# TGoldC/Motion-Planning-for-Autonomous-Driving-with-MPC

Measured on AMD Instinct MI355X. Metric: MPC steps/sec (N=30, nx=6 nu=2) at batch=4096, higher is better.
Workload: dtype f64; 1 GPU; N=30 nx=6 nu=2 bicycle lane-following, batch=4096/GPU, tol 1e-8; mode=converged, gpu=AMD Radeon Graphics

## Files before the change

motion-planning-for-autonomous-driving-with-mpc_amd/csrc/mpc_host_common.h:

```cpp
#pragma once
#include <cmath>
#include <cstddef>
#include <cstdint>
#include <cstdio>
#include <string>
#include <utility>
#include <vector>

#include "../../include/mpcgpu.h"
#include "mpc_stage_math.h"

namespace mpc {

constexpr double BOUND_RELAX = 1e-8;
constexpr int SENS_NWT = 7, SENS_NWQ = 5;
constexpr int LOOP_NS = 5, LOOP_NPOSE = 3;

struct HostProblem {
    mpc_problem_desc desc{};
    std::vector<double> LB, UB;
    int has_fl = 0, has_fu = 0, has_ol = 0, has_ou = 0;
    double fl = 0, fu = 0, ol = 0, ou = 0;
    double ol_raw = 0;
    double fl_raw = 0;
// ... 146 lines not shown
    w.MZU = w.total; w.total += mb * NZ;
    w.MSO = w.total; w.total += mb * 4;
    w.MNUO = w.total; w.total += mb * 4;
    w.MZLO = w.total; w.total += mb * 4;
    w.MZUO = w.total; w.total += mb * 4;
    w.MLAM = w.total; w.total += mb * XS;
    w.MREF = w.total; w.total += mb * XS;
    w.itotal = w.ntiles * w.itile_elems;
    return w;
}

inline int pick_bx(int N, int max_threads) {
    int bx = 64;
    while (bx > 4 && bx * (N + 1) > max_threads) bx >>= 1;
    return bx;
}

inline int dec_s_of(const HostProblem& hp) {
    return (hp.desc.nx == 6 && hp.desc.Q[5] == 0.0 && !((hp.lo_mask | hp.hi_mask) & (1u << 7))) ? 1 : 0;
}

inline void fill_params(Params& P, const HostProblem& hp, int B, size_t Bp, int bx, double* base, int32_t* ibase,
                        const double* dLB, const double* dUB, bool mailbox = true, int obst_stages = 0) {
    const mpc_problem_desc& d = hp.desc;
    const WsLayout w = ws_layout(d.N, d.nx, Bp, mailbox, obst_stages);
    P.B = B; P.Bp = (int32_t)Bp; P.N = d.N; P.nx = d.nx; P.bx = bx;
    P.obst_mult = d.obst_mult; P.max_iter = d.max_iter; P.fixed_iters = d.fixed_iters;
    P.has_fl = hp.has_fl; P.has_fu = hp.has_fu; P.has_ol = hp.has_ol; P.has_ou = hp.has_ou; P.per_inst_obst = OBST_SHARED;
    P.dt = d.dt; P.wheelbase = d.wheelbase; P.friction_div = d.friction_div; P.ego_offset = d.ego_offset; P.tol = d.tol;
    for (int i = 0; i < 6; ++i) P.Q[i] = (i < d.nx) ? d.Q[i] : 0.0;
    P.R[0] = d.R[0]; P.R[1] = d.R[1];
    for (int i = 0; i < 6; ++i) P.obst[i] = d.obstacle[i];
    P.fl = hp.fl; P.fu = hp.fu; P.ol = hp.ol; P.ou = hp.ou;
    P.inv_S = (uint32_t)((0x100000000ull + (uint64_t)d.N) / (uint64_t)(d.N + 1));
    P.run_counter = nullptr;
    P.dec_s = 0;
    P.tile_mask = nullptr;
    P.lo_mask = hp.lo_mask; P.hi_mask = hp.hi_mask; P.dense_mask = hp.dense_mask;
    P.dec_s = dec_s_of(hp);
    P.x0 = nullptr; P.p = nullptr; P.LB = dLB; P.UB = dUB;
    P.Z = base + w.Z * 64; P.ZL = base + w.ZL * 64; P.ZU = base + w.ZU * 64;
    P.SO = base + w.SO * 64; P.NUO = base + w.NUO * 64; P.ZLO = base + w.ZLO * 64; P.ZUO = base + w.ZUO * 64;
    P.LAM = base + w.LAM * 64; P.REF = base + w.REF * 64; P.DZ = base + w.DZ * 64; P.PK = base + w.PK * 64; P.KK = base + w.KK * 64;
    P.BLK = base + w.BLK * 64; P.ROLL = base + w.ROLL * 64; P.SC = base + w.SC * 64;
    P.FILT = base + w.FILT * 64; P.OBST = base + w.OBST * 64;
    P.MBLK = base + w.MBLK; P.MPK = base + w.MPK; P.MDZ = base + w.MDZ;
    P.MZ = base + w.MZ; P.MZL = base + w.MZL; P.MZU = base + w.MZU; P.MSO = base + w.MSO; P.MNUO = base + w.MNUO; P.MZLO = base + w.MZLO;
    P.MZUO = base + w.MZUO; P.MLAM = base + w.MLAM; P.MREF = base + w.MREF;
    P.tile_elems = (uint32_t)w.tile_elems; P.itile_elems = (uint32_t)w.itile_elems;
    P.ISC = ibase;
    P.WS = base; P.IWS = ibase;
    P.ws_bytes = (uint32_t)(w.total * sizeof(double)); P.iws_bytes = (uint32_t)(w.itotal * sizeof(int32_t));
    P.x_out = nullptr; P.status_out = nullptr; P.iters_out = nullptr; P.kkt_out = nullptr;
    P.emit = 0; P.fail_count = nullptr; P.fin_ctl = nullptr; P.fin_host = nullptr;
    P.DBG = nullptr;
    P.tile0 = 0;
}

inline void default_desc(mpc_problem_desc* d, int32_t N, int32_t nx) {
    *d = mpc_problem_desc{};
    d->N = N; d->nx = nx; d->nu = 2; d->formulation = MPC_FORM_CASADI_EULER;
    d->max_iter = 100; d->fixed_iters = 0; d->obst_mult = 3; d->device = 0;
    d->dt = 0.1; d->wheelbase = 2.5789128; d->friction_div = 2.578; d->ego_offset = 0.75; d->tol = 1e-8;
    const double Q[5] = {2.3, 2.3, 500.0, 0.1, 10.0};
    for (int i = 0; i < 5; ++i) d->Q[i] = Q[i];
    d->R[0] = 2.0; d->R[1] = 0.2;
    const double Pt[5] = {80.0, 80.0, 100.0, 0.1, 100.0};
    for (int i = 0; i < 5; ++i) d->P[i] = Pt[i];
    for (int j = 0; j < 3; ++j) { d->obstacle[2 * j] = -100.0; d->obstacle[2 * j + 1] = 0.0; }
}

}
```

motion-planning-for-autonomous-driving-with-mpc_amd/csrc/mpc_solve_plan.h:

```cpp
#pragma once
#include <algorithm>
#include <cctype>
#include <cstdlib>
#include <cstring>
#include <string>

#include "mpc_host_common.h"

namespace mpc {

struct Knobs {
    int pipeline, hybrid, hybrid_bx, hybrid_live, pipe_help, pipe_test_abort, pipe_xcd_mask, pipe_early;
    int rescue, rescue_wg, rescue_alone, loop_async, sync_spin, max_batch, friction_lb, bound_mask, big_wg, groups, poison;
    int timing;
    Knobs();
};
enum class KnobParse {
    ON,
    INT,
    FLAG,
    MASK,
    FRIC,
};
struct KnobDef { const char* name; int Knobs::*field; int dflt; KnobParse parse; };
inline constexpr KnobDef KNOBS[] = {
    {"pipeline", &Knobs::pipeline, 1, KnobParse::ON},           {"hybrid", &Knobs::hybrid, 1, KnobParse::INT},
    {"hybrid_bx", &Knobs::hybrid_bx, 0, KnobParse::INT},        {"hybrid_live", &Knobs::hybrid_live, -1, KnobParse::INT},
    {"pipe_help", &Knobs::pipe_help, -1, KnobParse::INT},       {"pipe_test_abort", &Knobs::pipe_test_abort, 0, KnobParse::FLAG},
    {"pipe_xcd_mask", &Knobs::pipe_xcd_mask, 0, KnobParse::MASK}, {"rescue", &Knobs::rescue, 1, KnobParse::ON},
    {"rescue_wg", &Knobs::rescue_wg, 1, KnobParse::INT},        {"rescue_alone", &Knobs::rescue_alone, 0, KnobParse::FLAG},
    {"loop_async", &Knobs::loop_async, 1, KnobParse::ON},       {"sync_spin", &Knobs::sync_spin, 1, KnobParse::ON},
    {"max_batch", &Knobs::max_batch, 0, KnobParse::INT},        {"friction_lb", &Knobs::friction_lb, 0, KnobParse::FRIC},
    {"bound_mask", &Knobs::bound_mask, 1, KnobParse::INT},      {"big_wg", &Knobs::big_wg, 0, KnobParse::FLAG},
    {"groups", &Knobs::groups, 0, KnobParse::INT},              {"poison", &Knobs::poison, 0, KnobParse::FLAG},
    {"timing", &Knobs::timing, 0, KnobParse::INT},               {"pipe_early", &Knobs::pipe_early, -1, KnobParse::INT},
};
inline Knobs::Knobs() { for (const KnobDef& e : KNOBS) this->*e.field = e.dflt; }
inline const KnobDef* find_knob(const char* name) {
    for (const KnobDef& e : KNOBS) if (name && strcmp(name, e.name) == 0) return &e;
    return nullptr;
}
inline int set_knob(Knobs& k, const char* name, const char* value) {
    const KnobDef* e = find_knob(name);
    if (!e) return MPC_ERR_INVALID;
    int v = e->dflt;
    if (value) {
        const long iv = strtol(value, nullptr, 0);
        switch (e->parse) {
            case KnobParse::ON: v = value[0] != '0'; break;
            case KnobParse::INT: v = (int)iv; break;
            case KnobParse::FLAG: v = (value[0] == '\0' ? 1 : (int)iv) != 0; break;
            case KnobParse::MASK: v = (int)(uint32_t)strtoul(value, nullptr, 0); break;
            case KnobParse::FRIC: v = strcmp(value, "ipopt") == 0 ? 1 : strcmp(value, "nlp") == 0 ? 0 : (int)iv; break;
        }
    }
    k.*e->field = v;
    return MPC_OK;
}
inline int get_knob(const Knobs& k, const char* name, long* out) {
    const KnobDef* e = find_knob(name);
    if (!e) return MPC_ERR_INVALID;
    *out = e->parse == KnobParse::MASK ? (long)(uint32_t)(k.*e->field) : (long)(k.*e->field);
    return MPC_OK;
}
inline void knobs_from_env(Knobs& k) {
    for (const KnobDef& e : KNOBS) {
        std::string env = "MPCGPU_";
        for (const char* c = e.name; *c; ++c) env += (char)toupper(*c);
        const char* v = getenv(env.c_str());
        if (v) (void)set_knob(k, e.name, v);
    }
}

constexpr int TIMING_STAGE = 1,
              TIMING_PIPE = 2,
              TIMING_WG = 4,
              TIMING_START = 8,
              TIMING_WG_TRACE = 16;

constexpr int STAGE_MAX_THREADS = 512;
constexpr int MAX_GROUPS = 4;
constexpr int MAX_POLL_IT = 1024;
constexpr size_t LDS_MAX = 160 * 1024 - 1024;

#ifndef MPC_STAGE_STASH
#define MPC_STAGE_STASH 1
#endif
template <int NX> struct Stash {
// ... 297 lines not shown
```

motion-planning-for-autonomous-driving-with-mpc_amd/csrc/mpc_stage_math.h:

```cpp
#pragma once
#include <math.h>
#include <stdint.h>

#if defined(__HIPCC__)
#define MPC_HD __host__ __device__ __forceinline__
#else
#define MPC_HD inline
#endif

#if defined(__HIP_DEVICE_COMPILE__)
#define MPC_GLOBAL_AS __attribute__((address_space(1)))
#else
#define MPC_GLOBAL_AS
#endif
#define MPC_GP(ptr, idx) (((MPC_GLOBAL_AS __typeof__(*(ptr))*)(ptr))[(uint32_t)(idx)])

namespace mpc {

constexpr double MU_INIT = 0.1, KAPPA_EPS = 10.0, KAPPA_MU = 0.2, THETA_MU = 1.5, TAU_MIN = 0.99;
constexpr double KAPPA_1 = 1e-2, KAPPA_2 = 1e-2, S_MAX = 100.0, KAPPA_SIGMA = 1e10;
constexpr double GAMMA_THETA = 1e-5, GAMMA_PHI = 1e-8, LS_DELTA = 1.0, S_THETA = 1.1, S_PHI = 2.3;
constexpr double ETA_PHI = 1e-8, GAMMA_ALPHA = 0.05;
constexpr double DW_MIN = 1e-20, DW_0 = 1e-4, DW_MAX = 1e40, KW_MINUS = 1.0 / 3.0, KW_PLUS = 8.0, KW_PLUS_BAR = 100.0;
constexpr double SCALING_MAX_GRAD = 100.0;
// ... 25 lines not shown
    SC_COUNT
};
enum IsRow { IS_STATUS = 0, IS_ITERS, IS_NFILT, IS_HAVETH0, IS_CONV, IS_ROLL, IS_FROW,
             IS_ILL,
             IS_RLEV, IS_ITACC,
             IS_COUNT };
enum ObstMode : int32_t { OBST_SHARED = 0, OBST_PER_INSTANCE = 1, OBST_PER_STAGE = 2, OBST_PER_STAGE_SIZED = 3 };
MPC_HD constexpr bool obst_mode_staged(int32_t m) { return m == OBST_PER_STAGE || m == OBST_PER_STAGE_SIZED; }
struct Params {
    int32_t B, Bp, N, nx, bx;
    int32_t obst_mult, max_iter, fixed_iters;
    int32_t has_fl, has_fu, has_ol, has_ou;
    int32_t per_inst_obst;
    double dt, wheelbase, friction_div, ego_offset, tol;
    double Q[6], R[2], obst[6];
    double fl, fu, ol, ou;
    int32_t dec_s;
    unsigned long long* tile_mask;
    int32_t* run_counter;
    uint32_t inv_S;
    uint32_t dense_mask;
    uint32_t lo_mask, hi_mask;
    const double* x0;
    const double* p;
    const double* LB;
    const double* UB;
    double *Z, *ZL, *ZU;
    double *SO, *NUO, *ZLO, *ZUO;
    double *LAM;
    double *REF;
    double *DZ;
    double *PK;
    double *KK;
    double *BLK;
    double *ROLL;
    double *MBLK, *MPK, *MDZ;
    double *MZ, *MZL, *MZU, *MSO, *MNUO, *MZLO, *MZUO, *MLAM, *MREF;
    double *SC;
    double *FILT;
    const double* OBST;
    int32_t* ISC;
    double* WS;
    int32_t* IWS;
    uint32_t ws_bytes, iws_bytes;
    uint32_t tile_elems, itile_elems;
    int32_t tile0;
    int32_t mbw_live;
    unsigned long long* DBG;
    double* x_out;
    int32_t* status_out;
    int32_t* iters_out;
    double* kkt_out;
    int32_t emit;
    uint32_t* fail_count;
    uint32_t *fin_ctl, *fin_host;
};

#define MPC_EV(R) ((((uint32_t)(R)) + 1u) & ~1u)
MPC_HD constexpr uint32_t mpc_prow(uint32_t r) { return (r & ~1u) * 64u + (r & 1u); }
MPC_HD uint32_t ws_index(const Params& P, const double*, uint32_t row, uint32_t b) { return (b >> 6) * P.tile_elems + mpc_prow(row) + (b & 63u) * 2u; }
MPC_HD uint32_t ws_index(const Params& P, const int32_t*, uint32_t row, uint32_t b) { return (b >> 6) * P.itile_elems + mpc_prow(row) + (b & 63u) * 2u; }

#if defined(__HIP_DEVICE_COMPILE__)
typedef unsigned int mpc_v2u __attribute__((ext_vector_type(2)));
__host__ __device__ __forceinline__ __amdgpu_buffer_rsrc_t mpc_rsrc(const void* base, uint32_t bytes) {
    const uint64_t a = (uint64_t)(uintptr_t)base;
    uint32_t lo = (uint32_t)__builtin_amdgcn_readfirstlane((int)(uint32_t)a);
    uint32_t hi = (uint32_t)__builtin_amdgcn_readfirstlane((int)(uint32_t)(a >> 32));
    bytes = (uint32_t)__builtin_amdgcn_readfirstlane((int)bytes);
    asm("" : "+s"(lo), "+s"(hi), "+s"(bytes));
    return __builtin_amdgcn_make_buffer_rsrc((void*)(uintptr_t)(((uint64_t)hi << 32) | lo), 0, (int)bytes, 0x00020000);
}
__device__ __forceinline__ int mpc_uni(uint32_t v) { return __builtin_amdgcn_readfirstlane((int)v); }
constexpr int MPC_AUX_SC1 = 16;
struct DevParams : Params {
    __amdgpu_buffer_rsrc_t rws, riws;
    bool xcu;
    __host__ __device__ __forceinline__ explicit DevParams(const Params& q, const bool xcu_ = false)
        : Params(q), rws(mpc_rsrc(q.WS, q.ws_bytes)), riws(mpc_rsrc(q.IWS, q.iws_bytes)), xcu(xcu_) {}
};
typedef DevParams PRef;
__device__ __forceinline__ PRef mpc_pref(const Params& q, const bool xcu) { return DevParams(q, xcu); }
__device__ __forceinline__ mpc_v2u mpc_bload64(const DevParams& P, const __amdgpu_buffer_rsrc_t r, const int voff, const int soff) {
    return P.xcu ? __builtin_amdgcn_raw_buffer_load_b64(r, voff, soff, MPC_AUX_SC1) : __builtin_amdgcn_raw_buffer_load_b64(r, voff, soff, 0);
}
__device__ __forceinline__ unsigned mpc_bload32(const DevParams& P, const __amdgpu_buffer_rsrc_t r, const int voff, const int soff) {
    return P.xcu ? __builtin_amdgcn_raw_buffer_load_b32(r, voff, soff, MPC_AUX_SC1) : __builtin_amdgcn_raw_buffer_load_b32(r, voff, soff, 0);
}
struct WsRefD {
    const PRef& P;
    uint32_t aoff, uoff, voff;
    __device__ __forceinline__ operator double() const {
        const __amdgpu_buffer_rsrc_t r = P.rws;
        const mpc_v2u v = mpc_bload64(P, r, (int)voff, mpc_uni(aoff + uoff));
        return __builtin_bit_cast(double, v);
    }
    __device__ __forceinline__ double operator=(double x) const {
        __builtin_amdgcn_raw_buffer_store_b64(__builtin_bit_cast(mpc_v2u, x), P.rws, (int)voff, mpc_uni(aoff + uoff), 0);
        return x;
    }
    __device__ __forceinline__ double operator=(const WsRefD& o) const { return (*this = (double)o); }
};
struct WsRefI {
    const PRef& P;
    uint32_t soff, voff;
    __device__ __forceinline__ operator int32_t() const {
// ... 2079 lines not shown
```

motion-planning-for-autonomous-driving-with-mpc_amd/csrc/mpcgpu.hip:

```cpp
#include <hip/hip_runtime.h>
#include <type_traits>

#include <algorithm>
#include <cctype>
#include <cstdio>
#include <cstdlib>
#include <cstring>
#include <new>
#include <string>
#include <vector>

#include "mpc_host_common.h"
#include "mpc_solve_plan.h"
#include "mpc_stamps.h"
#include "mpc_closed_loop.h"
#include "mpc_forces_qp.h"
#include "mpc_riccati_mfma.h"
#include "mpc_sens.h"
#include "mpc_loop_lin.h"

using namespace mpc;

namespace {

__device__ __forceinline__ void lds_barrier() {
    asm volatile("s_waitcnt lgkmcnt(0)\n\ts_barrier" ::: "memory");
}
template <int MAXJ, class Load, class Store>
__device__ __forceinline__ void batched_fill(const int n, const int t, const int NT, Load ld, Store st) {
    for (int q0 = 0; q0 < n; q0 += MAXJ * NT) {
        double v[MAXJ];
#pragma unroll
        for (int j = 0; j < MAXJ; ++j) { const int q = q0 + j * NT + t; v[j] = (q < n) ? (double)ld(q) : 0.0; }
#pragma unroll
        for (int j = 0; j < MAXJ; ++j) { const int q = q0 + j * NT + t; if (q < n) st(q, v[j]); }
    }
}
template <int MAXJ>
__device__ __forceinline__ void fill_bounds(const PRef& P, double* tab, const int nb, const int t, const int NT) {
    batched_fill<2 * MAXJ>(2 * nb, t, NT, [&](int q) { return q < nb ? (double)MPC_GP(P.LB, q) : (double)MPC_GP(P.UB, q - nb); }, [&](int q, double v) { tab[q] = v; });
}

__device__ __forceinline__ uint32_t lds_uniform(const uint32_t v) { return (uint32_t)__builtin_amdgcn_readfirstlane((int)v); }
__device__ __forceinline__ int lds_uniform(const int v) { return __builtin_amdgcn_readfirstlane(v); }
__device__ __forceinline__ double lds_uniform(const double v) {
    const unsigned long long u = __builtin_bit_cast(unsigned long long, v);
    const unsigned long long r = ((unsigned long long)lds_uniform((uint32_t)(u >> 32)) << 32) | lds_uniform((uint32_t)u);
    return __builtin_bit_cast(double, r);
}

template <typename R>
__device__ __forceinline__ R shfl_xor_struct(const R& r, int mask) {
    constexpr int NQ = sizeof(R) / sizeof(double);
    R o;
    const double* s = reinterpret_cast<const double*>(&r);
    double* d = reinterpret_cast<double*>(&o);
#pragma unroll
    for (int i = 0; i < NQ; ++i) d[i] = __shfl_xor(s[i], mask, 64);
    return o;
}

template <typename R>
__device__ __forceinline__ void block_reduce(R& r, int bx, double* lds) {
    constexpr int NQ = sizeof(R) / sizeof(double);
    for (int m = bx; m < 64; m <<= 1) {
        const R o = shfl_xor_struct(r, m);
        red_combine(r, o);
    }
    const int nw = blockDim.x >> 6;
    if (nw > 1) {
        const int wave = threadIdx.x >> 6, lane = threadIdx.x & 63, bl = lane & (bx - 1);
        double* mine = reinterpret_cast<double*>(&r);
        if (lane < bx) {
#pragma unroll
            for (int q = 0; q < NQ; ++q) lds[(wave * NQ + q) * bx + lane] = mine[q];
        }
        lds_barrier();
        R acc;
        double* a = reinterpret_cast<double*>(&acc);
#pragma unroll
        for (int q = 0; q < NQ; ++q) a[q] = lds[q * bx + bl];
        for (int w = 1; w < nw; ++w) {
            R o;
            double* op = reinterpret_cast<double*>(&o);
#pragma unroll
            for (int q = 0; q < NQ; ++q) op[q] = lds[(w * NQ + q) * bx + bl];
            red_combine(acc, o);
        }
        r = acc;
        lds_barrier();
    }
}

typedef __attribute__((address_space(3))) void* lds_ptr_t;
template <int NX, bool OUT, uint32_t VM = 0xFFu>
__device__ __forceinline__ void stash_xfer(Ctx<NX>& c, double* st, int T, int t, bool has_ou) {
    int r = 0;
#define MPC_ST(v) do { if (OUT) st[r * T + t] = (v); else (v) = st[r * T + t]; ++r; } while (0)
#pragma unroll
    for (int i = 0; i < NX + 2; ++i) { if (!((VM >> i) & 1u)) continue; MPC_ST(c.zl[i]); MPC_ST(c.zu[i]); MPC_ST(c.igl[i]); MPC_ST(c.igu[i]); }
#pragma unroll
    for (int j = 0; j < 3; ++j) { MPC_ST(c.zlo[j]); MPC_ST(c.iglo[j]); }
    if (has_ou) {
#pragma unroll
        for (int j = 0; j < 3; ++j) { MPC_ST(c.zuo[j]); MPC_ST(c.iguo[j]); }
    }
#pragma unroll
    for (int j = 0; j < 3; ++j) MPC_ST(c.nuo[j]);
#pragma unroll
    for (int i = 0; i < NX; ++i) { MPC_ST(c.lam[i]); MPC_ST(c.dlam[i]); }
#undef MPC_ST
}

#ifndef MPC_REF_FLAGS
#define MPC_REF_FLAGS (VM_OSPEC | vm_dense(REF_DENSE_LO, REF_DENSE_HI))
#endif
constexpr uint32_t REF_VM = REF_BOUND_VM | MPC_REF_FLAGS;
constexpr uint32_t SIZED_VM = 0xFFu | VM_SIZED;
constexpr uint32_t var_vm(int var) { return var == 2 ? REF_VM : var == 4 ? SIZED_VM : 0xFFu; }
struct NoStepWait {
    __device__ __forceinline__ bool there() const { return true; }
    __device__ __forceinline__ bool operator()() const { return true; }
};
template <int NX, bool INIT, int MAXT, uint32_t VM = 0xFFu, class StepWait = NoStepWait, bool OSTG = true>
__device__ __forceinline__ void stage_block(const PRef& P, const int n_mult, const int n_z, const int stash_rows, const uint32_t b0,
                                            const unsigned long long tile_bits, double* lds, const bool stamp = true,
                                            uint32_t* live_out = nullptr, const bool bounds_in_lds = false, const StepWait& step_wait = StepWait()) {
    constexpr bool EARLY = !std::is_same<StepWait, NoStepWait>::value;
    static_assert(!(EARLY && INIT), "the start iterate reads no step");
    CtxOf<NX, VM> c;
    constexpr bool STASH = MAXT <= 256 && MPC_STAGE_STASH;
    const bool has_ou = (VM & VM_OSPEC) ? false : (P.has_ou != 0);
    const int bx = P.bx, t = threadIdx.x;
    c.k = t / bx;
    c.b = (int)b0 + (t & (bx - 1));
    c.valid = (c.k <= P.N) && (c.b < P.B);
    c.active = false;
    c.ill = false;
    c.status = 0;
    c.iters = 0;
    c.mbw = !INIT && P.mbw_live > 0 && __popcll(tile_bits) <= P.mbw_live;
    MPC_STAMP(P.DBG, blockIdx.x, SB_ENTER, t == 0 && stamp);
    if (!INIT) {
        const unsigned long long m = tile_bits >> (b0 & 63u);
        if ((m & ((bx >= 64) ? ~0ull : ((1ull << bx) - 1ull))) == 0ull) return;
    }
    double* lds_b = lds + (blockDim.x >> 6) * 10 * bx;
    const int nb = (P.N + 1) * (NX + 2);
    double* lds_x = lds_b + 2 * nb;
    if (!bounds_in_lds)
        fill_bounds<2>(P, lds_b, nb, t, (int)blockDim.x);
    c.bnd = (mpc_lds_cptr)(lds_ptr_t)lds_b;
    c.bnd_ub = nb;
    if (INIT) lds_barrier();
    if (INIT) {
        Red0 r0;
        phase_init_point<NX, OSTG, (VM & VM_SIZED) != 0u>(P, c, r0);
        block_reduce(r0, bx, lds);
        phase_init_scalars<NX>(P, c, r0);
    } else {
        phase_load_scalars<NX>(P, c);
        PreTmp<NX> tmp;
        if constexpr (EARLY) {
            phase_preload<NX, false, VM, true, false, false>(P, c, tmp);
            if (step_wait.there()) {
                phase_preload_step<NX>(P, c);
                MPC_STAMP(P.DBG, blockIdx.x, SB_ISSUED, t == 0 && stamp);
            } else {
                MPC_STAMP(P.DBG, blockIdx.x, SB_ISSUED, t == 0 && stamp);
                if (!step_wait()) return;
                phase_preload_step<NX>(P, c);
            }
            phase_premath<NX, VM>(P, c, tmp);
        } else {
            phase_preload<NX, false, VM>(P, c, tmp);
            phase_premath<NX, VM>(P, c, tmp);
            MPC_STAMP(P.DBG, blockIdx.x, SB_ISSUED, t == 0 && stamp);
        }
        if (P.emit && c.valid && c.status == ST_SWEEP_FAILED) {
            emit_result<NX>(P, c, -7, c.iters, c.k == 0 ? (double)MPC_S(P.SC, SC_E0) : 0.0);
            if (c.k == 0) MPC_S(P.ISC, IS_STATUS) = -7;
        }
        if (!bounds_in_lds) lds_barrier();
        if (!__any(c.active ? 1 : 0)) return;
        MPC_STAMP(P.DBG, blockIdx.x, SB_LOADED, t == 0 && stamp);
        Red1 r1;
        phase_step_candidates<NX, VM>(P, c, r1);
        MPC_STAMP(P.DBG, blockIdx.x, SB_P1, t == 0 && stamp);
        block_reduce(r1, bx, lds);
        phase_linesearch_begin<NX>(P, c, r1);
        MPC_STAMP(P.DBG, blockIdx.x, SB_RED1, t == 0 && stamp);
        double* stash = lds_x;
        if (STASH) stash_xfer<NX, true, VM>(c, stash, blockDim.x, t, has_ou);
        while (__any((c.active && c.searching) ? 1 : 0)) {
            Red2 r2;
            phase_trial_eval<NX, VM>(P, c, r2);
            block_reduce(r2, bx, lds);
            phase_linesearch_decide<NX>(P, c, r2);
        }
        if (STASH) stash_xfer<NX, false, VM>(c, stash, blockDim.x, t, has_ou);
        MPC_STAMP(P.DBG, blockIdx.x, SB_LS, t == 0 && stamp);
        phase_apply_update<NX, false, VM>(P, c);
        MPC_STAMP(P.DBG, blockIdx.x, SB_UPDATE, t == 0 && stamp);
    }
    {
        double* ex = lds_x;
        const int T = blockDim.x;
#pragma unroll
        for (int i = 0; i < NX; ++i) { ex[i * T + t] = c.z[2 + i]; ex[(NX + i) * T + t] = c.lam[i]; }
        lds_barrier();
        const int tn = t + bx;
        if (tn < T) {
#pragma unroll
            for (int i = 0; i < NX; ++i) { c.xn[i] = ex[i * T + tn]; c.lamn[i] = ex[(NX + i) * T + tn]; }
        }
    }
    MPC_STAMP(P.DBG, blockIdx.x, SB_XCHG, t == 0 && stamp);
    Red3 r3;
    phase_eval_assemble<NX, !INIT, false, VM>(P, c, r3);
    MPC_STAMP(P.DBG, blockIdx.x, SB_EVAL, t == 0 && stamp);
    block_reduce(r3, bx, lds);
    MPC_STAMP(P.DBG, blockIdx.x, SB_RED3, t == 0 && stamp);
    phase_finish<NX, false>(P, c, r3, n_mult, n_z);
    MPC_STAMP(P.DBG, blockIdx.x, SB_END, t == 0 && stamp);
    if (live_out != nullptr && t < 64) {
        const unsigned long long m = __ballot((c.valid && c.k == 0 && c.active && c.status == ST_RUNNING) ? 1 : 0);
        if (t == 0) *live_out = (uint32_t)m;
    }
    if (P.run_counter != nullptr && t < 64) {
        const int cnt = __popcll(__ballot((c.valid && c.k == 0 && c.active && c.status == ST_RUNNING) ? 1 : 0));
        if (t == 0 && cnt) atomicAdd(P.run_counter, cnt);
    }
}

struct WgIo { uint32_t fail; uint32_t ill; double* c0; double* rn; double* r0; double* scl; bool fric, have; };
template <int NX, uint32_t VM, class Mid>
__device__ __forceinline__ void wg_stage(const PRef& P, const int ib0, const int ib1, double* lds_bnd, const mpc_lds_ptr rec_base, const int n_mult, const int n_z, const bool stamp,
                                         uint32_t* live_out, WgIo& io, Mid&& mid) {
    const int bx = P.bx, t = threadIdx.x;
    CtxOf<NX, VM> c;
    PreTmp<NX> tmp;
    c.k = t / bx;
    c.bl = t & (bx - 1);
    c.mb = (int)blockIdx.x * bx;
    c.b = c.bl ? ib1 : ib0;
    c.valid = (c.k <= P.N) && (c.b >= 0) && (c.b < P.B);
    c.active = false;
    c.ill = false;
    c.status = 0;
    c.iters = 0;
    c.rec = rec_base + ((t & (bx - 1)) * (P.N + 1) + (c.k <= P.N ? c.k : 0)) * Rec<NX>::SIZE;
    c.bnd = (mpc_lds_cptr)(lds_ptr_t)lds_bnd;
    c.bnd_ub = (P.N + 1) * (NX + 2);
    c.scl = (mpc_lds_ptr)(lds_ptr_t)(io.scl + c.bl * WgScl::SIZE);
    mid();
    phase_load_scalars<NX, true>(P, c);
    if (io.have) {
        phase_preload<NX, true, VM, false, true>(P, c, tmp, io.fric);
#pragma unroll
        for (int i = 0; i < NX; ++i) { c.rn[i] = io.rn[t * NX + i]; c.r0[i] = c.k == 0 ? io.r0[c.bl * 8 + i] : 0.0; }
    } else {
        phase_preload<NX, true, VM, false>(P, c, tmp);
#pragma unroll
        for (int i = 0; i < NX; ++i) { io.rn[t * NX + i] = c.rn[i]; if (c.k == 0 && c.valid) io.r0[c.bl * 8 + i] = c.r0[i]; }
        io.fric = __ballot((c.valid && c.k == 0 && c.fric_row) ? 1 : 0) != 0ull;
    }
    MPC_STAMP(P.DBG, blockIdx.x, SB_ENTER, t == 0 && stamp);
    if (((io.fail >> (t & (bx - 1))) & 1u) && c.valid) { c.status = -7; c.active = false; }
    phase_preload_rec<NX>(P, c, tmp);
    phase_premath<NX, VM>(P, c, tmp);
    MPC_STAMP(P.DBG, blockIdx.x, SB_ISSUED, t == 0 && stamp);
    if (!__any(c.active ? 1 : 0)) return;
    MPC_STAMP(P.DBG, blockIdx.x, SB_LOADED, t == 0 && stamp);
    Red1 r1;
// ... 546 lines not shown
                        if (t == 0) {
                            pipe_add(stage_done + pipe_item_tile(item), 1u);
                            ++n_help;
                        }
                    }
                    lds_barrier();
                }
            }
            if (all_done) break;
        }
        if (t == 0) { atomicAdd(reinterpret_cast<unsigned long long*>(A.ctl + PIPE_STATS) + P64_RIC_WAIT, waited); pipe_add(abort_w + PH_RIC_WORKERS, 1u); if (n_help) pipe_add(abort_w + PH_HELPED, n_help); }
        return;
    }
    unsigned long long busy = 0;
    uint32_t n_items = 0;
    bool have_bounds = false;
    for (;;) {
        MPC_STAMP(P.DBG, blockIdx.x, PW_TAKE, t == 0 && n_pass == 5u);
        if (t == 0) {
            const uint32_t tk = pipe_add(X + PX_HEAD, 1u);
            const unsigned long long* sl = slots + (tk & (A.cap - 1u));
            uint32_t item = PIPE_EXIT;
            const unsigned long long t0 = wall_clock64();
            for (;;) {
                const unsigned long long v = __hip_atomic_load(sl, __ATOMIC_RELAXED, __HIP_MEMORY_SCOPE_AGENT);
                if ((uint32_t)(v >> 32) == tk + 1u) { item = (uint32_t)v; break; }
                if (pipe_ld(X + PX_FINISHED) >= n_tiles_x || pipe_ld(abort_w)) break;
                if (wall_clock64() - t0 > PIPE_SPIN_LIMIT) { pipe_st(abort_w + PH_DETAIL, tk); pipe_st(abort_w + PH_DETAIL + 1, pipe_ld(X + PX_TAIL)); pipe_st(abort_w + PH_DETAIL + 3, (uint32_t)(wall_clock64() - t0)); pipe_st(abort_w, 4u); break; }
                __builtin_amdgcn_s_sleep(MPC_PIPE_SLEEP);
            }
            const unsigned long long t1 = wall_clock64();
            MPC_STAMP(P.DBG, blockIdx.x, PW_GOT, t == 0 && n_pass == 5u);
            waited += t1 - t0;
            busy -= t1;
            unsigned long long bits = 0ull;
            if (item != PIPE_EXIT) {
                bits = __hip_atomic_load(P.tile_mask + pipe_item_tile(item), __ATOMIC_RELAXED, __HIP_MEMORY_SCOPE_AGENT);
                pipe_acquire();
                asm volatile("s_waitcnt vmcnt(0)" ::: "memory");
            }
            sh_word[1] = item;
            sh_word[2] = (uint32_t)bits;
            sh_word[3] = (uint32_t)(bits >> 32);
        }
        lds_barrier();
        const uint32_t item = lds_uniform(sh_word[1]);
        const unsigned long long bits = ((unsigned long long)lds_uniform(sh_word[3]) << 32) | lds_uniform(sh_word[2]);
        if (item == PIPE_EXIT) break;
        MPC_STAMP(P.DBG, blockIdx.x, PW_BCAST, t == 0 && n_pass == 5u);
        const uint32_t tile = pipe_item_tile(item);
        if constexpr (HELP)
            stage_block<NX, false, 256, var_vm(VAR)>(P, n_mult, n_z, stash_rows, tile * 64u + pipe_item_q(item) * (uint32_t)P.bx, bits, lds, n_pass == 5u, nullptr, have_bounds);
        else
            stage_block<NX, false, 256, var_vm(VAR)>(P, n_mult, n_z, stash_rows, tile * 64u + pipe_item_q(item) * (uint32_t)P.bx, bits, lds, n_pass == 5u, nullptr, have_bounds,
                                                                   PipeStepWait{step_ready + tile, abort_w, &sh_word[0], pipe_item_round(item), tile, kpub < 0});
        have_bounds = have_bounds || ((bits >> ((pipe_item_q(item) * (uint32_t)P.bx) & 63u)) & ((P.bx >= 64) ? ~0ull : ((1ull << P.bx) - 1ull))) != 0ull;
        asm volatile("s_waitcnt vmcnt(0)" ::: "memory");
        lds_barrier();
        MPC_STAMP(P.DBG, blockIdx.x, PW_DONE, t == 0 && n_pass == 5u);
        if (t == 0) {
            pipe_add(stage_done + tile, 1u);
            busy += wall_clock64();
            ++n_items;
        }
        MPC_STAMP(P.DBG, blockIdx.x, PW_SIGNALLED, t == 0 && n_pass == 5u);
        ++n_pass;
    }
    if (A.ho_list != nullptr && t < 64 && pipe_ld(abort_w) == 0u) {
        pipe_acquire();
        asm volatile("s_waitcnt vmcnt(0)" ::: "memory");
        for (;;) {
            uint32_t j = 0u;
            if (t == 0) j = pipe_add(X + PX_HO_TICKET, 1u);
            j = (uint32_t)__builtin_amdgcn_readfirstlane((int)j);
            if (j >= n_tiles_x) break;
            ho_lists(P, (j * n_xcd + xcd) * 64u + (uint32_t)t, A.ho_list, A.ctl + PIPE_HO, stage_done);
        }
    }
    if (t == 0) {
        unsigned long long* st = reinterpret_cast<unsigned long long*>(A.ctl + PIPE_STATS);
        atomicAdd(st + P64_STAGE_WAIT, waited);
        atomicAdd(st + P64_STAGE_BUSY, busy + wall_clock64());
        atomicAdd(st + P64_ITEMS, (unsigned long long)n_items);
        pipe_add(abort_w + PH_STAGE_WORKERS, 1u);
    }
#endif
}

struct PrestartFromWs {
    __device__ __forceinline__ double z(int, int, int) const { return 0.0; }
    __device__ __forceinline__ double ref0(int, int) const { return 0.0; }
};
template <int NX, class Src = PrestartFromWs> __device__ __forceinline__ void prestart_par_block(const PRef& P, const uint32_t b0, double* sm, const Src src = Src{});

template <int NX, bool OSTG = false>
__device__ __attribute__((noinline)) void wg_restart(const PRef& Pin, const int n_mult, const int n_z, const int stash_rows, const uint32_t b0, double* lds,
                                                     uint32_t* live_out, const bool carry, const bool from_xs, const bool keep_first, const bool first_tiled) {
    const PRef P = mpc_pref(static_cast<const Params&>(Pin), false);
    using D = Dim<NX>;
    const int t = threadIdx.x, N = P.N, bx = P.bx;
    struct { int b, k, mb, bl; } c;
    c.k = t / bx;
    c.bl = t & (bx - 1);
    c.mb = (int)blockIdx.x * bx;
    c.b = (int)b0 + c.bl;
    const bool valid = (c.k <= N) && (c.b < P.B);
    if (valid) {
// ... 2301 lines not shown
            const auto kf = start_kernel<NX>(P.per_inst_obst);
            hipLaunchKernelGGL(kf, dim3(q.nblk), dim3(pl.threads), pl.lds_start, q.st, Pg, h->hp.n_mult, h->hp.n_z, pl.stash_rows,
                               g == 0 ? zero_next : (uint32_t*)nullptr, (uint32_t)ctl_words);
            if (g == 0 && zero_next != nullptr) next_zeroed = true;
            if (Pg.DBG) (void)report_stamps(Pg.DBG, (size_t)STAMP_SLOTS * q.nblk, [&](const unsigned long long* r) { return format_start_timing(r, q.nblk); }, q.st);
        } else {
            hipLaunchKernelGGL((k_ingest<NX>), dim3(q.ntl, (n_w + 63) / 64 + (n_w - 2 * d.N + 63) / 64), dim3(256), 0, q.st, Pg);
            hipLaunchKernelGGL((k_prestart_par<NX>), dim3(q.nblk), dim3(pl.threads), pl.lds_pre, q.st, Pg);
            launch_stage<NX>(s, q, true);
        }
        if (G > 1) s.prof.end(q.st);
    }
    if (s.ctl != nullptr) {
        h->pipe_clean[h->pipe_flip ^ 1] = next_zeroed ? ctl_words : 0;
        h->pipe_flip ^= 1;
    }
    return MPC_OK;
}

template <int NX> static int solve_wg_alone(Solve& s) {
    mpc_handle* h = s.h; const SolvePlan& pl = s.pl;
    DevTmp t_rdbg;
    if (pl.wg_timing) HIP_TRY(h, stamp_rows(t_rdbg, pl.wg_grid, s.stream));
    s.P.DBG = t_rdbg.as<unsigned long long>();
    s.prof.next(5, s.stream);
    launch_wg<NX>(s, nullptr, nullptr);
    s.prof.end(s.stream);
    s.out.mode = 2;
    if (s.call.async) {
        HIP_TRY(h, hipGetLastError());
        s.out.async_ok = true;
        return MPC_OK;
    }
    HIP_TRY(h, wait_stream(h, s.stream));
    read_head(s);
    if (s.t_wtrace.p) (void)report_stamps(s.t_wtrace.as<unsigned long long>(), (size_t)4 * s.n_wtrace, [&](const unsigned long long* r) { return format_wg_trace(r, s.n_wtrace); });
    if (s.P.DBG) HIP_TRY(h, report_stamps(s.P.DBG, (size_t)STAMP_SLOTS * pl.wg_grid, [&](const unsigned long long* r) { return format_wg_timing(r, pl.wg_grid); }));
    s.P.DBG = nullptr;
    return MPC_OK;
}

constexpr int PIPE_ABANDONED = -1000;
template <int NX> static int solve_pipeline(Solve& s) {
    mpc_handle* h = s.h; const SolvePlan& pl = s.pl;
    hipStream_t stream = s.stream; Params& P = s.P;
    int32_t* ho_list = pl.hand > 0 ? static_cast<int32_t*>(scratch_get(h, SCR_HO_LIST, (size_t)HO_BUCKETS * pl.ntiles * 64 * sizeof(int32_t))) : nullptr;
    if (pl.hand > 0 && !ho_list) { h->err = "out of device memory"; return MPC_ERR_HIP; }
    const PipeArgs A{s.ctl, (uint32_t)pl.ntiles, pl.xcd_mask, (uint32_t)pl.n_ric, pl.pipe_cap, 64u / (uint32_t)pl.bx, (uint32_t)pl.hand, ho_list, h->knobs.pipe_test_abort ? 2u : 0u, (uint32_t)pl.pipe_lead};
    DevTmp t_pdbg;
    if (pl.pipe_timing) HIP_TRY(h, stamp_rows(t_pdbg, h->n_cu, stream));
    P.DBG = t_pdbg.as<unsigned long long>();
    s.prof.next(3, stream);
    P.mbw_live = pl.mbw_live;
    const auto kf = pipeline_kernel<NX>(pl.pipe_help, pl.masked, pl.sized);
    hipLaunchKernelGGL(kf, dim3(h->n_cu), dim3(pl.threads), std::max(pl.lds_bytes, pl.ric_lds), stream, P, A, h->hp.n_mult, h->hp.n_z, pl.stash_rows);
    if (pl.hand > 0) {
        if (!h->prof_span) s.prof.next(5, stream);
        launch_wg<NX>(s, (const uint32_t*)(s.ctl + PIPE_ABORT), A.ho_list);
    }
    s.prof.end(stream);
    if (s.call.async) {
        hipLaunchKernelGGL(k_loop_sticky, dim3(1), dim3(1), 0, stream, (const uint32_t*)(s.ctl + PIPE_ABORT), h->d_fail + FAIL_LOOP_ABORT);
        HIP_TRY(h, hipGetLastError());
        s.out.async_ok = true;
        s.out.mode = 1;
        return MPC_OK;
    }
    if (pl.hand <= 0) HIP_TRY(h, hipMemcpyAsync(h->h_pipe, s.ctl + PIPE_ABORT, PH_WORDS * sizeof(uint32_t), hipMemcpyDeviceToHost, stream));
    HIP_TRY(h, wait_stream(h, stream));
    if (s.t_wtrace.p) (void)report_stamps(s.t_wtrace.as<unsigned long long>(), (size_t)4 * s.n_wtrace, [&](const unsigned long long* r) { return format_wg_trace(r, s.n_wtrace); });
    read_head(s);
    const uint32_t* hd = h->h_pipe;
    if (hd[PH_ABORT] != 0u) {
        h->pipe_disabled = true;
        fprintf(stderr, "[mpcgpu] single-launch pipeline abandoned (bounded wait expired: code %u, %u / %u, a millisecond later %u, waited %u ticks); re-running with one launch per kernel\n",
                hd[PH_ABORT], hd[PH_DETAIL], hd[PH_DETAIL + 1], hd[PH_DETAIL + 2], hd[PH_DETAIL + 3]);
        report_arrivals(s.ctl, pl.ntiles, A.items);
        return PIPE_ABANDONED;
    }
    P.DBG = nullptr;
    if (t_pdbg.p) HIP_TRY(h, report_stamps(t_pdbg.as<unsigned long long>(), (size_t)STAMP_SLOTS * h->n_cu, [&](const unsigned long long* r) { return format_pipe_timing(r, h->n_cu); }));
    s.out.mode = 1;
    return MPC_OK;
}

static int record_trace(const Solve& s, int row, double* d_trace) {
    double* const trace = s.io.trace.out;
    if (!trace || row >= s.io.trace.rows) return MPC_OK;
    hipLaunchKernelGGL(k_gather_trace, dim3((s.io.B + 255) / 256), dim3(256), 0, s.stream, s.h->d_ws + s.w.SC * 64, (uint32_t)s.w.tile_elems, s.io.B, d_trace);
    HIP_TRY(s.h, hipStreamSynchronize(s.stream));
    HIP_TRY(s.h, hipMemcpy(trace + (size_t)row * 8 * s.io.B, d_trace, sizeof(double) * 8 * (size_t)s.io.B, hipMemcpyDeviceToHost));
    return MPC_OK;
}
template <int NX> static int solve_per_kernel(Solve& s) {
    mpc_handle* h = s.h; const bool trace = s.io.trace.out != nullptr;
    const mpc_problem_desc& d = h->hp.desc;
    const SolvePlan& pl = s.pl;
    const int B = s.io.B, G = pl.G, nblk = pl.nblk;
    hipStream_t stream = s.stream; Params& P = s.P;
    int& it = s.out.iters;
    DevTmp t_trace, t_dbg;
    if (trace) HIP_TRY(h, hipMalloc(&t_trace.p, sizeof(double) * 8 * (size_t)B));
    if (pl.stage_timing) HIP_TRY(h, stamp_rows(t_dbg, nblk, stream));
    unsigned long long* const d_dbg = t_dbg.as<unsigned long long>();
    if (!s.call.async) HIP_TRY(h, hipMemsetAsync(h->d_fail + FAIL_COUNT, 0, sizeof(uint32_t), stream));
    if (pl.polled) HIP_TRY(h, hipMemsetAsync(h->d_counter, 0, sizeof(int32_t) * MAX_GROUPS * MAX_POLL_IT, stream));
// ... 1382 lines not shown
```

Before: 5.792 million MPC steps/s.

## Add transposed LDS block reduction for Red3 in pipeline stage

Adds a transposed block reduction for the Red3 struct. Each thread writes its fields into padded LDS columns grouped by operator (sum, min or max), then one wavefront per operator folds a column of per-wave partials with vectorised LDS loads, instead of the generic per-field block_reduce. It is enabled by default through a new red_transpose knob and only applies in the non-helper pipeline stage_block when bx==8, the block has 192 to 256 threads, and the stash has enough spare LDS. The aim is fewer barriers and serial reduction passes, at the cost of extra LDS use and an added branch.

```diff
diff --git a/motion-planning-for-autonomous-driving-with-mpc_amd/csrc/mpc_host_common.h b/motion-planning-for-autonomous-driving-with-mpc_amd/csrc/mpc_host_common.h
--- a/motion-planning-for-autonomous-driving-with-mpc_amd/csrc/mpc_host_common.h
+++ b/motion-planning-for-autonomous-driving-with-mpc_amd/csrc/mpc_host_common.h
@@ -222,7 +222,7 @@
     P.WS = base; P.IWS = ibase;
     P.ws_bytes = (uint32_t)(w.total * sizeof(double)); P.iws_bytes = (uint32_t)(w.itotal * sizeof(int32_t));
     P.x_out = nullptr; P.status_out = nullptr; P.iters_out = nullptr; P.kkt_out = nullptr;
-    P.emit = 0; P.fail_count = nullptr; P.fin_ctl = nullptr; P.fin_host = nullptr;
+    P.emit = 0; P.red_t = 0; P.fail_count = nullptr; P.fin_ctl = nullptr; P.fin_host = nullptr;
     P.DBG = nullptr;
     P.tile0 = 0;
 }
diff --git a/motion-planning-for-autonomous-driving-with-mpc_amd/csrc/mpc_red_fold.h b/motion-planning-for-autonomous-driving-with-mpc_amd/csrc/mpc_red_fold.h
--- /dev/null
+++ b/motion-planning-for-autonomous-driving-with-mpc_amd/csrc/mpc_red_fold.h
@@ -0,0 +1,50 @@
+#pragma once
+
+#include "mpc_stage_math.h"
+
+namespace mpc {
+
+enum RedOp : int { RED_SUM = 0, RED_MIN = 1, RED_MAX = 2 };
+MPC_HD constexpr int red_kind(const Red0*, int) { return RED_MAX; }
+MPC_HD constexpr int red_kind(const Red1*, int q) { return q < 2 ? RED_MIN : RED_SUM; }
+MPC_HD constexpr int red_kind(const Red2*, int q) { return q < 3 ? RED_SUM : RED_MAX; }
+MPC_HD constexpr int red_kind(const Red3*, int q) { return q == 2 ? RED_MIN : (q >= 4 && q <= 8) ? RED_SUM : RED_MAX; }
+template <int KIND> MPC_HD double red_op(double a, double b) {
+    if constexpr (KIND == RED_SUM) return a + b;
+    else if constexpr (KIND == RED_MIN) return fmin(a, b);
+    else return fmax(a, b);
+}
+
+template <class R> MPC_HD R red_fold_tree(const R* leaves, int len) {
+    if (len == 1) return leaves[0];
+    R a = red_fold_tree(leaves, len / 2);
+    const R b = red_fold_tree(leaves + len / 2, len / 2);
+    red_combine(a, b);
+    return a;
+}
+template <class R> MPC_HD R red_fold(const R* leaves, int bx, int nwaves) {
+    const int W = 64 / bx;
+    R acc = red_fold_tree(leaves, W);
+    for (int w = 1; w < nwaves; ++w) {
+        const R o = red_fold_tree(leaves + w * W, W);
+        red_combine(acc, o);
+    }
+    return acc;
+}
+
+template <int KIND, int LEN, class Leaf> MPC_HD double red_tree_field(const int lo, Leaf&& leaf) {
+    if constexpr (LEN == 1) {
+        return leaf(lo);
+    } else {
+        const double a = red_tree_field<KIND, LEN / 2>(lo, leaf);
+        const double b = red_tree_field<KIND, LEN / 2>(lo + LEN / 2, leaf);
+        return red_op<KIND>(a, b);
+    }
+}
+template <int KIND, int W, class Leaf> MPC_HD double red_fold_field(const int nwaves, Leaf&& leaf) {
+    double acc = red_tree_field<KIND, W>(0, leaf);
+    for (int w = 1; w < nwaves; ++w) acc = red_op<KIND>(acc, red_tree_field<KIND, W>(w * W, leaf));
+    return acc;
+}
+
+}
diff --git a/motion-planning-for-autonomous-driving-with-mpc_amd/csrc/mpc_solve_plan.h b/motion-planning-for-autonomous-driving-with-mpc_amd/csrc/mpc_solve_plan.h
--- a/motion-planning-for-autonomous-driving-with-mpc_amd/csrc/mpc_solve_plan.h
+++ b/motion-planning-for-autonomous-driving-with-mpc_amd/csrc/mpc_solve_plan.h
@@ -13,6 +13,7 @@
     int pipeline, hybrid, hybrid_bx, hybrid_live, pipe_help, pipe_test_abort, pipe_xcd_mask, pipe_early;
     int rescue, rescue_wg, rescue_alone, loop_async, sync_spin, max_batch, friction_lb, bound_mask, big_wg, groups, poison;
     int timing;
+    int red_transpose;
     Knobs();
 };
 enum class KnobParse {
@@ -34,6 +35,7 @@
     {"bound_mask", &Knobs::bound_mask, 1, KnobParse::INT},      {"big_wg", &Knobs::big_wg, 0, KnobParse::FLAG},
     {"groups", &Knobs::groups, 0, KnobParse::INT},              {"poison", &Knobs::poison, 0, KnobParse::FLAG},
     {"timing", &Knobs::timing, 0, KnobParse::INT},               {"pipe_early", &Knobs::pipe_early, -1, KnobParse::INT},
+    {"red_transpose", &Knobs::red_transpose, 1, KnobParse::ON},
 };
 inline Knobs::Knobs() { for (const KnobDef& e : KNOBS) this->*e.field = e.dflt; }
 inline const KnobDef* find_knob(const char* name) {
diff --git a/motion-planning-for-autonomous-driving-with-mpc_amd/csrc/mpc_stage_math.h b/motion-planning-for-autonomous-driving-with-mpc_amd/csrc/mpc_stage_math.h
--- a/motion-planning-for-autonomous-driving-with-mpc_amd/csrc/mpc_stage_math.h
+++ b/motion-planning-for-autonomous-driving-with-mpc_amd/csrc/mpc_stage_math.h
@@ -101,6 +101,7 @@
     int32_t* iters_out;
     double* kkt_out;
     int32_t emit;
+    int32_t red_t;
     uint32_t* fail_count;
     uint32_t *fin_ctl, *fin_host;
 };
diff --git a/motion-planning-for-autonomous-driving-with-mpc_amd/csrc/mpcgpu.hip b/motion-planning-for-autonomous-driving-with-mpc_amd/csrc/mpcgpu.hip
--- a/motion-planning-for-autonomous-driving-with-mpc_amd/csrc/mpcgpu.hip
+++ b/motion-planning-for-autonomous-driving-with-mpc_amd/csrc/mpcgpu.hip
@@ -18,6 +18,7 @@
 #include "mpc_riccati_mfma.h"
 #include "mpc_sens.h"
 #include "mpc_loop_lin.h"
+#include "mpc_red_fold.h"
 
 using namespace mpc;
 
@@ -90,6 +91,66 @@
         r = acc;
         lds_barrier();
     }
+}
+
+constexpr int RED_CS = 34;
+constexpr int red_t_doubles(int nq, int bx) { return nq * bx * (RED_CS + 1); }
+template <typename R> constexpr int red_count(int kind) {
+    int n = 0;
+    for (int q = 0; q < (int)(sizeof(R) / sizeof(double)); ++q) n += red_kind((const R*)nullptr, q) == kind ? 1 : 0;
+    return n;
+}
+template <typename R> constexpr int red_base(int kind) { return kind == RED_SUM ? 0 : kind == RED_MIN ? red_count<R>(RED_SUM) : red_count<R>(RED_SUM) + red_count<R>(RED_MIN); }
+template <typename R> constexpr int red_row(int q) {
+    const int kind = red_kind((const R*)nullptr, q);
+    int n = red_base<R>(kind);
+    for (int i = 0; i < q; ++i) n += red_kind((const R*)nullptr, i) == kind ? 1 : 0;
+    return n;
+}
+typedef double mpc_d2 __attribute__((ext_vector_type(2)));
+template <int KIND>
+__device__ __forceinline__ double red_fold_column(const double* col, const int nw) {
+    double x[32];
+#pragma unroll
+    for (int s = 0; s < 32; s += 2) { const mpc_d2 v = *reinterpret_cast<const mpc_d2*>(col + s); x[s] = v.x; x[s + 1] = v.y; }
+    auto leaf = [&](const int s) { return x[s]; };
+    double acc = red_tree_field<KIND, 8>(0, leaf);
+#pragma unroll
+    for (int w = 1; w < 4; ++w)
+        if (w < nw) acc = red_op<KIND>(acc, red_tree_field<KIND, 8>(8 * w, leaf));
+    return acc;
+}
+template <typename R>
+__device__ __forceinline__ void block_reduce_t(R& r, double* scr) {
+    constexpr int NQ = sizeof(R) / sizeof(double), BX = 8;
+    static_assert(red_count<R>(RED_SUM) <= 8 && red_count<R>(RED_MIN) <= 8 && red_count<R>(RED_MAX) <= 8, "the fields of one operator fit one wavefront");
+    static_assert(RED_SUM == 0 && RED_MIN == 1 && RED_MAX == 2, "wavefront w folds operator w");
+    const int t = threadIdx.x, nw = blockDim.x >> 6, lane = t & 63, bl = t & (BX - 1);
+    const int wave = lds_uniform(t >> 6);
+    double* v = reinterpret_cast<double*>(&r);
+    double* res = scr + NQ * BX * RED_CS;
+    {
+        double* mine = scr + bl * RED_CS + (t >> 3);
+#pragma unroll
+        for (int q = 0; q < NQ; ++q) mine[red_row<R>(q) * BX * RED_CS] = v[q];
+    }
+    lds_barrier();
+    if (wave < 3) {
+        const int cnt = wave == RED_SUM ? red_count<R>(RED_SUM) : wave == RED_MIN ? red_count<R>(RED_MIN) : red_count<R>(RED_MAX);
+        const int base = wave == RED_SUM ? red_base<R>(RED_SUM) : wave == RED_MIN ? red_base<R>(RED_MIN) : red_base<R>(RED_MAX);
+        if (lane < cnt * BX) {
+            const int slot = base * BX + lane;
+            const double* col = scr + slot * RED_CS;
+            double out;
+            if (wave == RED_SUM) out = red_fold_column<RED_SUM>(col, nw);
+            else if (wave == RED_MIN) out = red_fold_column<RED_MIN>(col, nw);
+            else out = red_fold_column<RED_MAX>(col, nw);
+            res[slot] = out;
+        }
+    }
+    lds_barrier();
+#pragma unroll
+    for (int q = 0; q < NQ; ++q) v[q] = res[red_row<R>(q) * BX + bl];
 }
 
 typedef __attribute__((address_space(3))) void* lds_ptr_t;
@@ -122,7 +183,7 @@
     __device__ __forceinline__ bool there() const { return true; }
     __device__ __forceinline__ bool operator()() const { return true; }
 };
-template <int NX, bool INIT, int MAXT, uint32_t VM = 0xFFu, class StepWait = NoStepWait, bool OSTG = true>
+template <int NX, bool INIT, int MAXT, uint32_t VM = 0xFFu, class StepWait = NoStepWait, bool OSTG = true, bool RT = false>
 __device__ __forceinline__ void stage_block(const PRef& P, const int n_mult, const int n_z, const int stash_rows, const uint32_t b0,
                                             const unsigned long long tile_bits, double* lds, const bool stamp = true,
                                             uint32_t* live_out = nullptr, const bool bounds_in_lds = false, const StepWait& step_wait = StepWait()) {
@@ -219,7 +280,14 @@
     Red3 r3;
     phase_eval_assemble<NX, !INIT, false, VM>(P, c, r3);
     MPC_STAMP(P.DBG, blockIdx.x, SB_EVAL, t == 0 && stamp);
-    block_reduce(r3, bx, lds);
+    if constexpr (RT && !INIT) {
+        const int T = blockDim.x;
+        const bool fits = bx == 8 && T >= 192 && T <= 256 && (stash_rows - 2 * NX) * T >= red_t_doubles(sizeof(Red3) / sizeof(double), 8);
+        if (P.red_t != 0 && fits) block_reduce_t(r3, lds_x + 2 * NX * T);
+        else block_reduce(r3, bx, lds);
+    } else {
+        block_reduce(r3, bx, lds);
+    }
     MPC_STAMP(P.DBG, blockIdx.x, SB_RED3, t == 0 && stamp);
     phase_finish<NX, false>(P, c, r3, n_mult, n_z);
     MPC_STAMP(P.DBG, blockIdx.x, SB_END, t == 0 && stamp);
@@ -872,7 +940,7 @@
         if constexpr (HELP)
             stage_block<NX, false, 256, var_vm(VAR)>(P, n_mult, n_z, stash_rows, tile * 64u + pipe_item_q(item) * (uint32_t)P.bx, bits, lds, n_pass == 5u, nullptr, have_bounds);
         else
-            stage_block<NX, false, 256, var_vm(VAR)>(P, n_mult, n_z, stash_rows, tile * 64u + pipe_item_q(item) * (uint32_t)P.bx, bits, lds, n_pass == 5u, nullptr, have_bounds,
+            stage_block<NX, false, 256, var_vm(VAR), PipeStepWait, true, true>(P, n_mult, n_z, stash_rows, tile * 64u + pipe_item_q(item) * (uint32_t)P.bx, bits, lds, n_pass == 5u, nullptr, have_bounds,
                                                                    PipeStepWait{step_ready + tile, abort_w, &sh_word[0], pipe_item_round(item), tile, kpub < 0});
         have_bounds = have_bounds || ((bits >> ((pipe_item_q(item) * (uint32_t)P.bx) & 63u)) & ((P.bx >= 64) ? ~0ull : ((1ull << P.bx) - 1ull))) != 0ull;
         asm volatile("s_waitcnt vmcnt(0)" ::: "memory");
@@ -3280,6 +3348,7 @@
     P.DBG = t_pdbg.as<unsigned long long>();
     s.prof.next(3, stream);
     P.mbw_live = pl.mbw_live;
+    P.red_t = h->knobs.red_transpose;
     const auto kf = pipeline_kernel<NX>(pl.pipe_help, pl.masked, pl.sized);
     hipLaunchKernelGGL(kf, dim3(h->n_cu), dim3(pl.threads), std::max(pl.lds_bytes, pl.ric_lds), stream, P, A, h->hp.n_mult, h->hp.n_z, pl.stash_rows);
     if (pl.hand > 0) {
```

New measurement: 5.866 million MPC steps/s (median of 6 runs). 1.3% higher.
